# strongbeamsprout/gloria-nlp-project

Measured on AMD Instinct MI355X. Metric: image-text pairs/sec (whole node), imagenome_pretrain bs=256, higher is better.
Workload: dtype bf16

## Files before the change

### gloria-nlp-project_amd/csrc/glr_attn.hip

```cpp
#include "glr_attn_common.h"

namespace {

__global__ void __launch_bounds__(AT_NT) k_attn_fwd(AttnParams p) {
  extern __shared__ __attribute__((aligned(16))) unsigned char smem[];
  const int tid = threadIdx.x, lane = tid & 63, wave = tid >> 6, l31 = lane & 31, h = lane >> 5;
  const int bh = blockIdx.x, b = bh / p.nh, hd = bh % p.nh;
  int L; size_t row_base;
  attn_rows(p, b, row_base, L);
  const int tp = p.tp, lk = (L + 15) & ~15, kt = lk >> 4, nkb = (L + 31) >> 5;
  unsigned char* Qs = smem;
  unsigned char* Ks = Qs + 128 * AT_RP;
  unsigned char* Vt = Ks + 128 * AT_RP;
  unsigned char* Ps = smem;
  float* kb = reinterpret_cast<float*>(Vt + 64 * tp);
  const size_t base = row_base * p.ld + (size_t)hd * 64;
  {
    uint4 rq[4], rk[4], rv[4];
    tile_load(p.q + base, p.ld, L, rq, tid);
    tile_load(p.k + base, p.ld, L, rk, tid);
    tile_load(p.v + base, p.ld, L, rv, tid);
    tile_store_rows(rq, Qs, tid);
    tile_store_rows(rk, Ks, tid);
    tile_store_transposed(rv, lk, Vt, tp, tid);
  }
  if (tid < 128) kb[tid] = (tid < L && (p.key_mask == nullptr || p.key_mask[(size_t)b * L + tid] != 0)) ? 0.f : -INFINITY;
  __syncthreads();
  const int row0 = 32 * wave;
  f32x16 acc[4];
#pragma unroll
  for (int j = 0; j < 4; ++j) zero16(acc[j]);
  if (row0 < L) gemm_rows64(acc, Qs, row0, Ks, nkb, l31, h);
  __syncthreads();
  if (row0 >= L) return;
  float kbv[4];
#pragma unroll
  for (int j = 0; j < 4; ++j) kbv[j] = kb[32 * j + l31];
  const bool drop = p.p_drop > 0.f;
  const unsigned thr16 = drop ? (unsigned)(p.p_drop * 65536.f + 0.5f) : 0u;
  const float inv_keep = drop ? 1.f / (1.f - p.p_drop) : 1.f;
  const float sl = p.scale * AT_LOG2E;
  unsigned char* slab = Ps + wave * 32 * AT_SP;
  unsigned mw0 = 0u, mw1 = 0u;
  unsigned hk0, hk1;
  hash_key(p, hk0, hk1);
#pragma unroll
  for (int q = 0; q < 16; ++q) {
    const int r = acc_row(q, h);
    float v[4], m = -INFINITY;
#pragma unroll
    for (int j = 0; j < 4; ++j) { v[j] = __builtin_fmaf(acc[j][q], sl, kbv[j]); m = fmaxf(m, v[j]); }
    m = half_max(m);
    const float ms = m == -INFINITY ? 0.f : m;
    float e[4], s = 0.f;
#pragma unroll
    for (int j = 0; j < 4; ++j) { e[j] = __builtin_amdgcn_exp2f(v[j] - ms); s += e[j]; }
    s = half_sum(s);
    const float inv = s > 0.f ? 1.f / s : 0.f;
    if (l31 == 0) p.lse[(size_t)bh * 128 + row0 + r] = (ms + __builtin_amdgcn_logf(fmaxf(s, 1e-37f))) * (1.f / AT_LOG2E);
    unsigned r01 = 0u, r23 = 0u;
    if (drop) {
      const unsigned ctr = (((unsigned)bh * 128u + (unsigned)(row0 + r)) * 32u + (unsigned)l31) * 2u;
      r01 = hash32(ctr, hk0, hk1);
      r23 = hash32(ctr + 1u, hk0, hk1);
    }
    const unsigned r16[4] = {r01 & 0xffffu, r01 >> 16, r23 & 0xffffu, r23 >> 16};
#pragma unroll
    for (int j = 0; j < 4; ++j) {
      const bool keepb = !drop || r16[j] >= thr16;
      if (drop) {
        const unsigned long long word = __ballot(keepb);
        if (lane == q * 4 + j) { mw0 = (unsigned)word; mw1 = (unsigned)(word >> 32); }
      }
      const float pd = keepb ? e[j] * inv * inv_keep : 0.f;
      *reinterpret_cast<unsigned short*>(slab + r * AT_SP + (32 * j + l31) * 2) = f2bf(pd);
    }
  }
  if (drop) {
    const int q = lane >> 2, j = lane & 3;
    const int r0 = row0 + acc_row(q, 0);
    p.keep[((size_t)bh * 128 + r0) * 4 + j] = mw0;
    p.keep[((size_t)bh * 128 + r0 + 4) * 4 + j] = mw1;
  }
  f32x16 out[2];
  zero16(out[0]); zero16(out[1]);
  gemm_tokens(out, slab, Vt, tp, kt, l31, h);
  store_rows(out, slab, tp, p.o + row_base * p.ld_o + (size_t)hd * 64, p.ld_o, row0, L, lane, l31, h);
}

__global__ void __launch_bounds__(AT_NT, 2) k_attn_bwd_q(AttnParams p) {
  extern __shared__ __attribute__((aligned(16))) unsigned char smem[];
  const int tid = threadIdx.x, lane = tid & 63, wave = tid >> 6, l31 = lane & 31, h = lane >> 5;
  const int bh = blockIdx.x, b = bh / p.nh, hd = bh % p.nh;
  int L; size_t row_base;
  attn_rows(p, b, row_base, L);
  const int tp = p.tp, lk = (L + 15) & ~15, kt = lk >> 4, nkb = (L + 31) >> 5;
  unsigned char* Ks = smem;
  unsigned char* Vs = Ks + 128 * AT_RP;
  unsigned char* Kt = Vs + 128 * AT_RP;
  unsigned char* Ps = smem;
  float* kb = reinterpret_cast<float*>(Kt + 64 * tp);
  float* lse = kb + 128;
  float* delta = lse + 128;
  unsigned* keep = reinterpret_cast<unsigned*>(delta + 128);
  const size_t base = row_base * p.ld + (size_t)hd * 64, base_o = row_base * p.ld_o + (size_t)hd * 64;
  const bool drop = p.p_drop > 0.f;
  const int row0 = 32 * wave;
  const bool active = row0 < L;
  bf16x8 fq[4], fg[4];
  {
    uint4 rk[4], rv[4];
    bf16x8 fo[4];
    tile_load(p.k + base, p.ld, L, rk, tid);
    tile_load(p.v + base, p.ld, L, rv, tid);
    frag_rows_load(p.q + base, p.ld, row0 + l31, L, h, fq);
    frag_rows_load(p.d_o + base_o, p.ld_o, row0 + l31, L, h, fg);
    frag_rows_load(p.o + base_o, p.ld_o, row0 + l31, L, h, fo);
    if (tid < 128) {
      kb[tid] = (tid < L && (p.key_mask == nullptr || p.key_mask[(size_t)b * L + tid] != 0)) ? 0.f : -INFINITY;
      lse[tid] = tid < L ? p.lse[(size_t)bh * 128 + tid] * AT_LOG2E : 0.f;
    }
    for (int i = tid; i < 512; i += AT_NT) keep[i] = (drop && (i >> 2) < L) ? p.keep[(size_t)bh * 512 + i] : 0xffffffffu;
    tile_store_rows(rk, Ks, tid);
    tile_store_rows(rv, Vs, tid);
    tile_store_transposed(rk, lk, Kt, tp, tid);
    float d = 0.f;
#pragma unroll
    for (int ks = 0; ks < 4; ++ks) d += dot8(__builtin_bit_cast(uint4, fg[ks]), __builtin_bit_cast(uint4, fo[ks]));
    d += __shfl_xor(d, 32, 64);
    if (h == 0) delta[row0 + l31] = d;
  }
  __syncthreads();
  f32x16 acc[4], acc2[4], out[2];
#pragma unroll
  for (int j = 0; j < 4; ++j) { zero16(acc[j]); zero16(acc2[j]); }
  if (active) {
    gemm_frag64(acc, fq, Ks, nkb, l31, h);
    gemm_frag64(acc2, fg, Vs, nkb, l31, h);
  }
  __syncthreads();
  if (!active) return;
  const float inv_keep = drop ? 1.f / (1.f - p.p_drop) : 1.f;
  const float sl = p.scale * AT_LOG2E;
  unsigned char* slab = Ps + wave * 32 * AT_SP;
  {
    float kbv[4];
#pragma unroll
    for (int j = 0; j < 4; ++j) kbv[j] = kb[32 * j + l31];
#pragma unroll
    for (int q = 0; q < 16; ++q) {
      const int r = acc_row(q, h);
      const float lr = lse[row0 + r], dl = delta[row0 + r];
      const uint4 kw = *reinterpret_cast<const uint4*>(keep + (row0 + r) * 4);
      const unsigned kwj[4] = {kw.x, kw.y, kw.z, kw.w};
#pragma unroll
      for (int j = 0; j < 4; ++j) {
        const float pr = __builtin_amdgcn_exp2f(__builtin_fmaf(acc[j][q], sl, kbv[j]) - lr);
        const float dp = ((kwj[j] >> l31) & 1u) ? acc2[j][q] * inv_keep : 0.f;
        *reinterpret_cast<unsigned short*>(slab + r * AT_SP + (32 * j + l31) * 2) = f2bf(pr * (dp - dl) * p.scale);
      }
    }
  }
  zero16(out[0]); zero16(out[1]);
  gemm_tokens(out, slab, Kt, tp, kt, l31, h);
  store_rows(out, slab, tp, p.dq + base, p.ld, row0, L, lane, l31, h);
}

__global__ void __launch_bounds__(AT_NT, 2) k_attn_bwd_kv(AttnParams p) {
  extern __shared__ __attribute__((aligned(16))) unsigned char smem[];
  const int tid = threadIdx.x, lane = tid & 63, wave = tid >> 6, l31 = lane & 31, h = lane >> 5;
  const int bh = blockIdx.x, b = bh / p.nh, hd = bh % p.nh;
  int L; size_t row_base;
  attn_rows(p, b, row_base, L);
  const int tp = p.tp, lk = (L + 15) & ~15, kt = lk >> 4, nkb = (L + 31) >> 5;
  unsigned char* Qs = smem;
  unsigned char* Gs = Qs + 128 * AT_RP;
  unsigned char* Qt = Gs + 128 * AT_RP;
  unsigned char* Gt = Qt + 64 * tp;
  unsigned char* Ps = smem;
  float* kb = reinterpret_cast<float*>(Gt + 64 * tp);
  float* lse = kb + 128;
  float* delta = lse + 128;
  unsigned* keep = reinterpret_cast<unsigned*>(delta + 256);
  const size_t base = row_base * p.ld + (size_t)hd * 64, base_o = row_base * p.ld_o + (size_t)hd * 64;
  const bool drop = p.p_drop > 0.f;
  const int row0 = 32 * wave;
  const bool active = row0 < L;
  bf16x8 fk[4], fv[4];
  {
    uint4 rq[4], rg[4], ro[4];
    tile_load(p.q + base, p.ld, L, rq, tid);
    tile_load(p.d_o + base_o, p.ld_o, L, rg, tid);
    tile_load(p.o + base_o, p.ld_o, L, ro, tid);
    frag_rows_load(p.k + base, p.ld, row0 + l31, L, h, fk);
    frag_rows_load(p.v + base, p.ld, row0 + l31, L, h, fv);
    if (tid < 128) {
      kb[tid] = (tid < L && (p.key_mask == nullptr || p.key_mask[(size_t)b * L + tid] != 0)) ? 0.f : -INFINITY;
      lse[tid] = tid < L ? p.lse[(size_t)bh * 128 + tid] * AT_LOG2E : 0.f;
    }
    for (int i = tid; i < 512; i += AT_NT) keep[i] = (drop && (i >> 2) < L) ? p.keep[(size_t)bh * 512 + i] : 0xffffffffu;
    tile_store_rows(rq, Qs, tid);
    tile_store_rows(rg, Gs, tid);
    tile_store_transposed(rq, lk, Qt, tp, tid);
    tile_store_transposed(rg, lk, Gt, tp, tid);
    delta[tid] = (dot8(rg[0], ro[0]) + dot8(rg[1], ro[1])) + (dot8(rg[2], ro[2]) + dot8(rg[3], ro[3]));
  }
  __syncthreads();
  f32x16 acc[4], acc2[4], out[2];
#pragma unroll
  for (int j = 0; j < 4; ++j) { zero16(acc[j]); zero16(acc2[j]); }
  float lq[4], dq_[4], kbk16[16];
  unsigned kwq[4];
  if (active) {
    gemm_frag64(acc, fk, Qs, nkb, l31, h);
    gemm_frag64(acc2, fv, Gs, nkb, l31, h);
  }
#pragma unroll
  for (int j = 0; j < 4; ++j) {
    lq[j] = lse[32 * j + l31];
    dq_[j] = delta[32 * j + l31] + delta[128 + 32 * j + l31];
    kwq[j] = keep[(32 * j + l31) * 4 + wave];
  }
#pragma unroll
  for (int q = 0; q < 16; ++q) kbk16[q] = kb[row0 + acc_row(q, h)];
  __syncthreads();
  if (!active) return;
  const float inv_keep = drop ? 1.f / (1.f - p.p_drop) : 1.f;
  const float sl = p.scale * AT_LOG2E;
  unsigned char* slab = Ps + wave * 32 * AT_SP;
#pragma unroll
  for (int q = 0; q < 16; ++q) {
    const int r = acc_row(q, h);
#pragma unroll
    for (int j = 0; j < 4; ++j) {
      const float pr = __builtin_amdgcn_exp2f(__builtin_fmaf(acc[j][q], sl, kbk16[q]) - lq[j]);
      const bool keepb = (kwq[j] >> r) & 1u;
      *reinterpret_cast<unsigned short*>(slab + r * AT_SP + (32 * j + l31) * 2) = f2bf(keepb ? pr * inv_keep : 0.f);
      const float dp = keepb ? acc2[j][q] * inv_keep : 0.f;
      acc2[j][q] = pr * (dp - dq_[j]) * p.scale;
    }
  }
  zero16(out[0]); zero16(out[1]);
  gemm_tokens(out, slab, Gt, tp, kt, l31, h);
  {
    f32x16 dvv[2] = {out[0], out[1]};
#pragma unroll
    for (int q = 0; q < 16; ++q) {
      const int r = acc_row(q, h);
#pragma unroll
      for (int j = 0; j < 4; ++j) *reinterpret_cast<unsigned short*>(slab + r * AT_SP + (32 * j + l31) * 2) = f2bf(acc2[j][q]);
    }
    zero16(out[0]); zero16(out[1]);
    gemm_tokens(out, slab, Qt, tp, kt, l31, h);
    store_rows(out, slab, tp, p.dk + base, p.ld, row0, L, lane, l31, h);
    store_rows(dvv, slab, tp, p.dv + base, p.ld, row0, L, lane, l31, h);
  }
}

size_t attn_lds_fwd(int L) { return (size_t)2 * 128 * AT_RP + (size_t)64 * attn_tp(L) + 512; }
size_t attn_lds_bwd_q(int L) { return (size_t)2 * 128 * AT_RP + (size_t)64 * attn_tp(L) + 3 * 512 + 2048; }
size_t attn_lds_bwd_kv(int L) { return (size_t)2 * 128 * AT_RP + (size_t)2 * 64 * attn_tp(L) + 4 * 512 + 2048; }
size_t attn_lds_bwd(int L) { return attn_lds_bwd_kv(L) > attn_lds_bwd_q(L) ? attn_lds_bwd_kv(L) : attn_lds_bwd_q(L); }

}

extern "C" int glr_attn_max_tokens(int backward) {
  for (int L = 128; L > 0; L -= 16)
    if ((backward ? attn_lds_bwd(L) : attn_lds_fwd(L)) <= 160 * 1024) return L;
  return 0;
}

static int attn_launch_fwd(const AttnParams& p, void* stream) {
  const int lds = (int)attn_lds_fwd(p.L);
  static GlrLdsAttr lds_fwd;
  if (glr_ensure_lds(lds_fwd, (const void*)k_attn_fwd, lds) != GLR_OK) return GLR_ELAUNCH;
  hipLaunchKernelGGL(k_attn_fwd, dim3(p.B * p.nh), dim3(AT_NT), lds, (hipStream_t)stream, p);
  GLR_CHECK_LAUNCH();
  return GLR_OK;
}
static int attn_launch_bwd(const AttnParams& p, void* stream) {
  const int lds_q = (int)attn_lds_bwd_q(p.L), lds_kv = (int)attn_lds_bwd_kv(p.L);
  static GlrLdsAttr lds_bq, lds_bkv;
  if (glr_ensure_lds(lds_bq, (const void*)k_attn_bwd_q, lds_q) != GLR_OK) return GLR_ELAUNCH;
  if (glr_ensure_lds(lds_bkv, (const void*)k_attn_bwd_kv, lds_kv) != GLR_OK) return GLR_ELAUNCH;
  hipLaunchKernelGGL(k_attn_bwd_q, dim3(p.B * p.nh), dim3(AT_NT), lds_q, (hipStream_t)stream, p);
  GLR_CHECK_LAUNCH();
  hipLaunchKernelGGL(k_attn_bwd_kv, dim3(p.B * p.nh), dim3(AT_NT), lds_kv, (hipStream_t)stream, p);
  GLR_CHECK_LAUNCH();
  return GLR_OK;
}
static int attn_rows_longest(const int32_t* rs, int B, int max_n) {
  int longest = 0;
  for (int b = 0; b < B; ++b) {
    const long long n = (long long)rs[b + 1] - rs[b];
    if (rs[b] < 0 || n < 1 || n > max_n) return 0;
    if ((int)n > longest) longest = (int)n;
  }
  return longest;
}

extern "C" int glr_attn_fwd(const void* q, const void* k, const void* v, const uint8_t* key_mask, int B, int n_heads, int L, int ld,
                            int ld_o, float scale, float p_drop, unsigned long long seed, unsigned long long offset,
                            const unsigned long long* rng_cell, void* o, float* lse, uint32_t* keep, void* stream) {
  AttnParams p;
  const int rc = attn_fill(p, q, k, v, key_mask, B, n_heads, L, ld, ld_o, scale, p_drop, seed, offset, 128);
  if (rc != GLR_OK) return rc;
  if (!o || !lse || (p_drop > 0.f && !keep) || L > glr_attn_max_tokens(0)) return GLR_EINVAL;
  p.o = (unsigned short*)o; p.lse = lse; p.keep = keep; p.rng = rng_cell;
  return attn_launch_fwd(p, stream);
}

extern "C" int glr_attn_bwd(const void* q, const void* k, const void* v, const void* o, const void* d_o, const uint8_t* key_mask,
                            const float* lse, const uint32_t* keep, int B, int n_heads, int L, int ld, int ld_o, float scale, float p_drop,
                            void* dq, void* dk, void* dv, void* stream) {
  AttnParams p;
  const int rc = attn_fill(p, q, k, v, key_mask, B, n_heads, L, ld, ld_o, scale, p_drop, 0, 0, 128);
  if (rc != GLR_OK) return rc;
  if (!o || !d_o || !lse || !dq || !dk || !dv || (p_drop > 0.f && !keep) || L > glr_attn_max_tokens(1)) return GLR_EINVAL;
  p.o = (unsigned short*)const_cast<void*>(o); p.d_o = (const unsigned short*)d_o; p.lse = const_cast<float*>(lse);
  p.keep = const_cast<unsigned*>(keep); p.dq = (unsigned short*)dq; p.dk = (unsigned short*)dk; p.dv = (unsigned short*)dv;
  return attn_launch_bwd(p, stream);
}

extern "C" int glr_attn_rows_fwd(const void* q, const void* k, const void* v, const int32_t* row_start, const int32_t* row_start_host,
                                 int B, int n_heads, int ld, int ld_o, float scale, float p_drop, unsigned long long seed,
                                 unsigned long long offset, const unsigned long long* rng_cell, void* o, float* lse, uint32_t* keep,
                                 void* stream) {
  if (!row_start || !row_start_host || B <= 0) return GLR_EINVAL;
  const int longest = attn_rows_longest(row_start_host, B, glr_attn_max_tokens(0));
  if (longest == 0) return GLR_EINVAL;
  AttnParams p;
  const int rc = attn_fill(p, q, k, v, nullptr, B, n_heads, longest, ld, ld_o, scale, p_drop, seed, offset, 128);
  if (rc != GLR_OK) return rc;
  if (!o || !lse || (p_drop > 0.f && !keep)) return GLR_EINVAL;
  p.o = (unsigned short*)o; p.lse = lse; p.keep = keep; p.rng = rng_cell; p.row_start = row_start;
  return attn_launch_fwd(p, stream);
}

extern "C" int glr_attn_rows_bwd(const void* q, const void* k, const void* v, const void* o, const void* d_o, const int32_t* row_start,
                                 const int32_t* row_start_host, const float* lse, const uint32_t* keep, int B, int n_heads, int ld,
                                 int ld_o, float scale, float p_drop, void* dq, void* dk, void* dv, void* stream) {
  if (!row_start || !row_start_host || B <= 0) return GLR_EINVAL;
  const int longest = attn_rows_longest(row_start_host, B, glr_attn_max_tokens(1));
  if (longest == 0) return GLR_EINVAL;
  AttnParams p;
  const int rc = attn_fill(p, q, k, v, nullptr, B, n_heads, longest, ld, ld_o, scale, p_drop, 0, 0, 128);
  if (rc != GLR_OK) return rc;
  if (!o || !d_o || !lse || !dq || !dk || !dv || (p_drop > 0.f && !keep)) return GLR_EINVAL;
  p.o = (unsigned short*)const_cast<void*>(o); p.d_o = (const unsigned short*)d_o; p.lse = const_cast<float*>(lse);
  p.keep = const_cast<unsigned*>(keep); p.dq = (unsigned short*)dq; p.dk = (unsigned short*)dk; p.dv = (unsigned short*)dv;
  p.row_start = row_start;
  return attn_launch_bwd(p, stream);
}
```

### gloria-nlp-project_amd/csrc/glr_attn_common.h

```cpp
#pragma once
#include "glr_common.h"

namespace {

constexpr int AT_NT = 256;
constexpr int AT_RP = 144;
constexpr int AT_SP = 272;
constexpr float AT_LOG2E = 1.4426950408889634f;

struct AttnParams {
  const unsigned short* q; const unsigned short* k; const unsigned short* v;
  const unsigned char* key_mask;
  int B, nh, L, ld, ld_o;
  float scale, p_drop;
  unsigned seed_lo, seed_hi, off_lo, off_hi;
  const unsigned long long* rng;
  unsigned short* o;
  float* lse;
  unsigned* keep;
  const unsigned short* d_o;
  unsigned short* dq; unsigned short* dk; unsigned short* dv;
  int tp;
  const int* row_start;
};
// ... 40 lines not shown
  for (int q = 0; q < 16; ++q) a[q] = 0.f;
}
__device__ __forceinline__ int acc_row(int q, int h) { return (q & 3) + 8 * (q >> 2) + 4 * h; }

__device__ __forceinline__ void tile_load(const unsigned short* g, int ld, int L, uint4 (&r)[4], int tid) {
#pragma unroll
  for (int t = 0; t < 4; ++t) {
    const int i = tid + AT_NT * t, row = i & 127, pc = i >> 7;
    r[t] = make_uint4(0u, 0u, 0u, 0u);
    if (row < L) r[t] = *reinterpret_cast<const uint4*>(g + (size_t)row * ld + pc * 8);
  }
}
__device__ __forceinline__ void tile_store_rows(const uint4 (&r)[4], unsigned char* dst, int tid) {
#pragma unroll
  for (int t = 0; t < 4; ++t) {
    const int i = tid + AT_NT * t, row = i & 127, pc = i >> 7;
    *reinterpret_cast<uint4*>(dst + row * AT_RP + pc * 16) = r[t];
  }
}
__device__ __forceinline__ void tile_store_transposed(const uint4 (&r)[4], int lk, unsigned char* dst, int tp, int tid) {
#pragma unroll
  for (int t = 0; t < 4; ++t) {
    const int i = tid + AT_NT * t, row = i & 127, pc = i >> 7;
    if (row < lk) {
      const unsigned w[4] = {r[t].x, r[t].y, r[t].z, r[t].w};
#pragma unroll
      for (int e = 0; e < 4; ++e) {
        *reinterpret_cast<unsigned short*>(dst + (pc * 8 + 2 * e) * tp + row * 2) = (unsigned short)(w[e] & 0xffffu);
        *reinterpret_cast<unsigned short*>(dst + (pc * 8 + 2 * e + 1) * tp + row * 2) = (unsigned short)(w[e] >> 16);
      }
    }
  }
}
__device__ __forceinline__ float dot8(const uint4 a, const uint4 c) {
  const unsigned aw[4] = {a.x, a.y, a.z, a.w}, cw[4] = {c.x, c.y, c.z, c.w};
  float d = 0.f;
#pragma unroll
  for (int e = 0; e < 4; ++e) {
    d = __builtin_fmaf(__uint_as_float(aw[e] << 16), __uint_as_float(cw[e] << 16), d);
    d = __builtin_fmaf(__uint_as_float(aw[e] & 0xffff0000u), __uint_as_float(cw[e] & 0xffff0000u), d);
  }
  return d;
}
__device__ __forceinline__ void gemm_rows64(f32x16 (&acc)[4], const unsigned char* A, int arow0, const unsigned char* Bm, int nblk,
                                            int l31, int h) {
#pragma unroll
  for (int ks = 0; ks < 4; ++ks) {
    const bf16x8 fa = ldf(A + (arow0 + l31) * AT_RP + ks * 32 + h * 16);
#pragma unroll
    for (int j = 0; j < 4; ++j)
      if (j < nblk) mma(fa, ldf(Bm + (32 * j + l31) * AT_RP + ks * 32 + h * 16), acc[j]);
  }
}
__device__ __forceinline__ void gemm_tokens(f32x16 (&out)[2], const unsigned char* slab, const unsigned char* Bt, int tp, int kt,
                                            int l31, int h) {
  for (int ks = 0; ks < kt; ++ks) {
    const bf16x8 fa = ldf(slab + l31 * AT_SP + ks * 32 + h * 16);
#pragma unroll
    for (int c = 0; c < 2; ++c) mma(fa, ldf(Bt + (32 * c + l31) * tp + ks * 32 + h * 16), out[c]);
  }
}
__device__ __forceinline__ void store_rows(const f32x16 (&out)[2], unsigned char* slab, int tp, unsigned short* g, int ld, int row0, int L,
                                           int lane, int l31, int h) {
#pragma unroll
  for (int c = 0; c < 2; ++c)
#pragma unroll
// ... 53 lines not shown
```

### gloria-nlp-project_amd/csrc/glr_lnorm.hip

```cpp
#include "glr_common.h"

namespace {

constexpr int LN_NT = 256;

struct U4 { unsigned x, y, z, w; };
__device__ __forceinline__ U4 philox4x32(unsigned c0, unsigned c1, unsigned c2, unsigned c3, unsigned k0, unsigned k1) {
#pragma unroll
  for (int r = 0; r < 10; ++r) {
    const unsigned hi0 = __umulhi(0xD2511F53u, c0), lo0 = 0xD2511F53u * c0;
    const unsigned hi1 = __umulhi(0xCD9E8D57u, c2), lo1 = 0xCD9E8D57u * c2;
    c0 = hi1 ^ c1 ^ k0; c1 = lo1; c2 = hi0 ^ c3 ^ k1; c3 = lo0;
    k0 += 0x9E3779B9u; k1 += 0xBB67AE85u;
  }
  return {c0, c1, c2, c3};
}
__device__ __forceinline__ float wave_sum_f(float v) {
#pragma unroll
  for (int m = 32; m >= 1; m >>= 1) v += __shfl_xor(v, m, 64);
  return v;
}
__device__ __forceinline__ void unpack4(const uint2 u, float (&f)[4]) {
  f[0] = __uint_as_float(u.x << 16); f[1] = __uint_as_float(u.x & 0xffff0000u);
  f[2] = __uint_as_float(u.y << 16); f[3] = __uint_as_float(u.y & 0xffff0000u);
// ... 135 lines not shown
        dg[i][c] = __builtin_fmaf(dv[c], x, dg[i][c]);
        db[i][c] += dv[c];
      }
    }
    const float m1 = wave_sum_f(s1) * (1.f / H), m2 = wave_sum_f(s2) * (1.f / H);
#pragma unroll
    for (int i = 0; i < NQ; ++i) {
      const int quad = lane + 64 * i;
      float dz[4], dh[4];
#pragma unroll
      for (int c = 0; c < 4; ++c) {
        dz[c] = rstd * (gd[i][c] - m1 - xh[i][c] * m2);
        dh[c] = ((keepbits[i] >> c) & 1u) ? dz[c] * inv_keep : 0.f;
        dhs[i][c] += dh[c];
      }
      *reinterpret_cast<float4*>(d_inp + row * H + 4 * quad) = make_float4(dz[0], dz[1], dz[2], dz[3]);
      *reinterpret_cast<uint2*>(d_h + row * H + 4 * quad) = pack4(dh);
    }
  }
  __shared__ float red[3][LN_NT / 64][H];
#pragma unroll
  for (int i = 0; i < NQ; ++i)
#pragma unroll
    for (int c = 0; c < 4; ++c) {
      red[0][wv][4 * (lane + 64 * i) + c] = dg[i][c];
      red[1][wv][4 * (lane + 64 * i) + c] = db[i][c];
      red[2][wv][4 * (lane + 64 * i) + c] = dhs[i][c];
    }
  __syncthreads();
  for (int col = threadIdx.x; col < H; col += LN_NT) {
    float a = 0.f, b = 0.f, e = 0.f;
#pragma unroll
    for (int k = 0; k < LN_NT / 64; ++k) { a += red[0][k][col]; b += red[1][k][col]; e += red[2][k][col]; }
    part[(size_t)col * gridDim.x + blockIdx.x] = a;
    part[((size_t)H + col) * gridDim.x + blockIdx.x] = b;
    part[((size_t)2 * H + col) * gridDim.x + blockIdx.x] = e;
  }
}

__global__ void __launch_bounds__(LN_NT) k_ln_finish(const float* __restrict__ part, int n_part, int H, float* __restrict__ dgamma,
                                                     float* __restrict__ dbeta, void* __restrict__ dhsum, int dhsum_bf16) {
  const int lane = threadIdx.x & 63;
  const int col = blockIdx.x * (LN_NT / 64) + (threadIdx.x >> 6);
  if (col >= H) return;
  float a = 0.f, b = 0.f, e = 0.f;
  for (int k = lane; k < n_part; k += 64) {
    a += part[(size_t)col * n_part + k];
    b += part[((size_t)H + col) * n_part + k];
    if (dhsum) e += part[((size_t)2 * H + col) * n_part + k];
  }
  a = wave_sum_f(a);
  b = wave_sum_f(b);
  e = wave_sum_f(e);
  if (lane == 0) {
    dgamma[col] = a;
    dbeta[col] = b;
    if (dhsum) {
      if (dhsum_bf16) reinterpret_cast<unsigned short*>(dhsum)[col] = f2bf(e);
      else reinterpret_cast<float*>(dhsum)[col] = e;
    }
  }
}

constexpr int CS_COLS = 256;
__global__ void __launch_bounds__(LN_NT) k_colsum(const unsigned short* __restrict__ x, long long R, int C, long long rows_per,
                                                   float* __restrict__ part) {
  const int ct = threadIdx.x & 31, rl = threadIdx.x >> 5;
  const int col0 = blockIdx.x * CS_COLS + ct * 8;
  const long long r0 = (long long)blockIdx.y * rows_per;
  const long long r1 = r0 + rows_per < R ? r0 + rows_per : R;
  float acc[8] = {0.f, 0.f, 0.f, 0.f, 0.f, 0.f, 0.f, 0.f};
  const unsigned short* px = x + col0;
  long long r = r0 + rl;
  for (; r + 24 < r1; r += 32) {
    uint4 v[4];
#pragma unroll
    for (int u = 0; u < 4; ++u) v[u] = *reinterpret_cast<const uint4*>(px + (r + 8 * u) * C);
#pragma unroll
    for (int u = 0; u < 4; ++u) {
      acc[0] += __uint_as_float(v[u].x << 16); acc[1] += __uint_as_float(v[u].x & 0xffff0000u);
      acc[2] += __uint_as_float(v[u].y << 16); acc[3] += __uint_as_float(v[u].y & 0xffff0000u);
      acc[4] += __uint_as_float(v[u].z << 16); acc[5] += __uint_as_float(v[u].z & 0xffff0000u);
      acc[6] += __uint_as_float(v[u].w << 16); acc[7] += __uint_as_float(v[u].w & 0xffff0000u);
    }
  }
  for (; r < r1; r += 8) {
    const uint4 v = *reinterpret_cast<const uint4*>(px + r * C);
    acc[0] += __uint_as_float(v.x << 16); acc[1] += __uint_as_float(v.x & 0xffff0000u);
    acc[2] += __uint_as_float(v.y << 16); acc[3] += __uint_as_float(v.y & 0xffff0000u);
    acc[4] += __uint_as_float(v.z << 16); acc[5] += __uint_as_float(v.z & 0xffff0000u);
    acc[6] += __uint_as_float(v.w << 16); acc[7] += __uint_as_float(v.w & 0xffff0000u);
  }
  __shared__ float red[8][CS_COLS + 8];
#pragma unroll
// ... 79 lines not shown
                                   unsigned long long* mask, void* stream) {
  return drop_add_ln_fwd(h16, inp32, gamma, beta, R, H, eps, p_drop, seed, offset, rng_cell, out32, out16, stats, mask, nullptr, stream);
}

extern "C" int glr_drop_add_ln_rows_fwd(const void* h16, const float* inp32, const float* gamma, const float* beta,
                                        const int32_t* row_ids, long long R, int H, float eps, float p_drop, unsigned long long seed,
                                        unsigned long long offset, const unsigned long long* rng_cell, float* out32, void* out16,
                                        float* stats, unsigned long long* mask, void* stream) {
  if (!row_ids) return GLR_EINVAL;
  return drop_add_ln_fwd(h16, inp32, gamma, beta, R, H, eps, p_drop, seed, offset, rng_cell, out32, out16, stats, mask, row_ids, stream);
}

extern "C" int glr_drop_add_ln_bwd(const float* dy32, const void* dy16, const void* h16, const float* inp32, const float* gamma,
                                   const float* stats, const unsigned long long* mask, long long R, int H, float p_drop,
                                   float* d_inp32, void* d_h16, float* workspace, float* dgamma, float* dbeta, void* dhsum,
                                   int dhsum_bf16, void* stream) {
  if ((!dy32 && !dy16) || !h16 || !inp32 || !gamma || !stats || !d_inp32 || !d_h16 || !workspace || !dgamma || !dbeta ||
      !ln_shape_ok(R, H))
    return GLR_EINVAL;
  if (p_drop < 0.f || p_drop >= 1.f || (p_drop > 0.f && !mask)) return GLR_EINVAL;
  hipStream_t st = (hipStream_t)stream;
  const int np = ln_parts(R);
#define GLR_LN_BWD(NQ)                                                                                                      \
  hipLaunchKernelGGL((k_drop_add_ln_bwd<NQ>), dim3(np), dim3(LN_NT), 0, st, dy32, (const unsigned short*)dy16,               \
                     (const unsigned short*)h16, inp32, gamma, stats, mask, R, p_drop, d_inp32, (unsigned short*)d_h16, workspace)
  switch (H / 256) {
    case 1: GLR_LN_BWD(1); break;
    case 2: GLR_LN_BWD(2); break;
    case 3: GLR_LN_BWD(3); break;
    default: GLR_LN_BWD(4); break;
  }
#undef GLR_LN_BWD
  GLR_CHECK_LAUNCH();
  hipLaunchKernelGGL(k_ln_finish, dim3((H + LN_NT / 64 - 1) / (LN_NT / 64)), dim3(LN_NT), 0, st, workspace, np, H, dgamma, dbeta, dhsum,
                     dhsum_bf16);
  GLR_CHECK_LAUNCH();
  return GLR_OK;
}
```

Baseline: 4102.

## Pack multiple short-sequence heads per attention block and restructure LN finish reduction

Attention forward and backward kernels now pack several heads into one 128-row block when the sequence is short (<=32 or <=64 tokens), using templated bodies that skip unused key blocks. This cuts idle waves and shrinks the grid for short text sequences. Separately, the layernorm-backward partials are stored row-major per block, and the finish kernel is rewritten as a column-coalesced 1024-thread reduction. The head packing adds index arithmetic and shared-memory layout complexity.

Result: slower. 4039 (-1.5%).

```diff
diff --git a/gloria-nlp-project_amd/csrc/glr_attn.hip b/gloria-nlp-project_amd/csrc/glr_attn.hip
--- a/gloria-nlp-project_amd/csrc/glr_attn.hip
+++ b/gloria-nlp-project_amd/csrc/glr_attn.hip
@@ -2,40 +2,66 @@
 
 namespace {
 
-__global__ void __launch_bounds__(AT_NT) k_attn_fwd(AttnParams p) {
-  extern __shared__ __attribute__((aligned(16))) unsigned char smem[];
+struct AttnUnit {
+  int hd, bh, hl, R0, row0, L, lk, kt, nkb, tp;
+  bool active;
+};
+__device__ __forceinline__ AttnUnit attn_unit(const AttnParams& p, int b, int hd0, int nhg, int sh, int L, int tp, int wave) {
+  AttnUnit u;
+  u.L = L; u.tp = tp;
+  u.R0 = 32 * wave; u.hl = u.R0 >> sh; u.row0 = u.R0 & ((1 << sh) - 1);
+  u.hd = hd0 + u.hl; u.bh = b * p.nh + u.hd;
+  u.lk = (L + 15) & ~15; u.kt = u.lk >> 4; u.nkb = (L + 31) >> 5;
+  u.active = u.hl < nhg && u.row0 < L;
+  return u;
+}
+__device__ __forceinline__ bool attn_group(const AttnParams& p, int G, int& b, int& hd0, int& nhg, int& sh, int& L, size_t& row_base, int& tp) {
+  b = blockIdx.x / G;
+  attn_rows(p, b, row_base, L);
+  sh = L <= 32 ? 5 : (L <= 64 ? 6 : 7);
+  const int hpw = 128 >> sh;
+  hd0 = (blockIdx.x % G) * hpw;
+  nhg = p.nh - hd0 < hpw ? p.nh - hd0 : hpw;
+  tp = (2 << sh) + 16;
+  return hd0 < p.nh;
+}
+
+template <int SH>
+__device__ __forceinline__ void attn_fwd_body(const AttnParams& p, unsigned char* smem, int b, int hd0, int nhg, int L_,
+                                              size_t row_base, int tp_) {
   const int tid = threadIdx.x, lane = tid & 63, wave = tid >> 6, l31 = lane & 31, h = lane >> 5;
-  const int bh = blockIdx.x, b = bh / p.nh, hd = bh % p.nh;
-  int L; size_t row_base;
-  attn_rows(p, b, row_base, L);
-  const int tp = p.tp, lk = (L + 15) & ~15, kt = lk >> 4, nkb = (L + 31) >> 5;
+  const AttnUnit u = attn_unit(p, b, hd0, nhg, SH, L_, tp_, wave);
+  constexpr int NKB = SH == 5 ? 1 : (SH == 6 ? 2 : 4);
+  const int L = u.L, tp = u.tp, lk = u.lk, kt = u.kt, nkb = NKB < 4 ? NKB : u.nkb, sh = SH, bh = u.bh, hd = u.hd;
   unsigned char* Qs = smem;
   unsigned char* Ks = Qs + 128 * AT_RP;
   unsigned char* Vt = Ks + 128 * AT_RP;
   unsigned char* Ps = smem;
-  float* kb = reinterpret_cast<float*>(Vt + 64 * tp);
-  const size_t base = row_base * p.ld + (size_t)hd * 64;
+  float* kb = reinterpret_cast<float*>(Vt + (64 * tp << (7 - sh)));
+  const size_t base = row_base * p.ld + (size_t)hd0 * 64;
   {
     uint4 rq[4], rk[4], rv[4];
-    tile_load(p.q + base, p.ld, L, rq, tid);
-    tile_load(p.k + base, p.ld, L, rk, tid);
-    tile_load(p.v + base, p.ld, L, rv, tid);
+    tile_load_group(p.q + base, p.ld, L, sh, nhg, rq, tid);
+    tile_load_group(p.k + base, p.ld, L, sh, nhg, rk, tid);
+    tile_load_group(p.v + base, p.ld, L, sh, nhg, rv, tid);
     tile_store_rows(rq, Qs, tid);
     tile_store_rows(rk, Ks, tid);
-    tile_store_transposed(rv, lk, Vt, tp, tid);
+    tile_store_transposed_group(rv, lk, Vt, tp, sh, tid);
   }
   if (tid < 128) kb[tid] = (tid < L && (p.key_mask == nullptr || p.key_mask[(size_t)b * L + tid] != 0)) ? 0.f : -INFINITY;
   __syncthreads();
-  const int row0 = 32 * wave;
+  Ks += (u.hl << sh) * AT_RP;
+  Vt += (size_t)u.hl * 64 * tp;
+  const int row0 = u.row0;
   f32x16 acc[4];
 #pragma unroll
   for (int j = 0; j < 4; ++j) zero16(acc[j]);
-  if (row0 < L) gemm_rows64(acc, Qs, row0, Ks, nkb, l31, h);
-  __syncthreads();
-  if (row0 >= L) return;
+  if (u.active) gemm_rows64(acc, Qs, u.R0, Ks, nkb, l31, h);
+  __syncthreads();
+  if (!u.active) return;
   float kbv[4];
 #pragma unroll
-  for (int j = 0; j < 4; ++j) kbv[j] = kb[32 * j + l31];
+  for (int j = 0; j < 4; ++j) kbv[j] = j < NKB ? kb[32 * j + l31] : -INFINITY;
   const bool drop = p.p_drop > 0.f;
   const unsigned thr16 = drop ? (unsigned)(p.p_drop * 65536.f + 0.5f) : 0u;
   const float inv_keep = drop ? 1.f / (1.f - p.p_drop) : 1.f;
@@ -49,12 +75,14 @@
     const int r = acc_row(q, h);
     float v[4], m = -INFINITY;
 #pragma unroll
-    for (int j = 0; j < 4; ++j) { v[j] = __builtin_fmaf(acc[j][q], sl, kbv[j]); m = fmaxf(m, v[j]); }
+    for (int j = 0; j < 4; ++j)
+      if (j < NKB) { v[j] = __builtin_fmaf(acc[j][q], sl, kbv[j]); m = fmaxf(m, v[j]); }
     m = half_max(m);
     const float ms = m == -INFINITY ? 0.f : m;
     float e[4], s = 0.f;
 #pragma unroll
-    for (int j = 0; j < 4; ++j) { e[j] = __builtin_amdgcn_exp2f(v[j] - ms); s += e[j]; }
+    for (int j = 0; j < 4; ++j)
+      if (j < NKB) { e[j] = __builtin_amdgcn_exp2f(v[j] - ms); s += e[j]; }
     s = half_sum(s);
     const float inv = s > 0.f ? 1.f / s : 0.f;
     if (l31 == 0) p.lse[(size_t)bh * 128 + row0 + r] = (ms + __builtin_amdgcn_logf(fmaxf(s, 1e-37f))) * (1.f / AT_LOG2E);
@@ -72,8 +100,10 @@
         const unsigned long long word = __ballot(keepb);
         if (lane == q * 4 + j) { mw0 = (unsigned)word; mw1 = (unsigned)(word >> 32); }
       }
-      const float pd = keepb ? e[j] * inv * inv_keep : 0.f;
-      *reinterpret_cast<unsigned short*>(slab + r * AT_SP + (32 * j + l31) * 2) = f2bf(pd);
+      if (j < NKB) {
+        const float pd = keepb ? e[j] * inv * inv_keep : 0.f;
+        *reinterpret_cast<unsigned short*>(slab + r * AT_SP + (32 * j + l31) * 2) = f2bf(pd);
+      }
     }
   }
   if (drop) {
@@ -88,49 +118,74 @@
   store_rows(out, slab, tp, p.o + row_base * p.ld_o + (size_t)hd * 64, p.ld_o, row0, L, lane, l31, h);
 }
 
-__global__ void __launch_bounds__(AT_NT, 2) k_attn_bwd_q(AttnParams p) {
-  extern __shared__ __attribute__((aligned(16))) unsigned char smem[];
-  const int tid = threadIdx.x, lane = tid & 63, wave = tid >> 6, l31 = lane & 31, h = lane >> 5;
-  const int bh = blockIdx.x, b = bh / p.nh, hd = bh % p.nh;
+__global__ void __launch_bounds__(AT_NT) k_attn_fwd(AttnParams p) {
+  extern __shared__ __attribute__((aligned(16))) unsigned char smem[];
+  const int b = blockIdx.x / p.nh, hd = blockIdx.x % p.nh;
   int L; size_t row_base;
   attn_rows(p, b, row_base, L);
-  const int tp = p.tp, lk = (L + 15) & ~15, kt = lk >> 4, nkb = (L + 31) >> 5;
+  attn_fwd_body<7>(p, smem, b, hd, 1, L, row_base, p.tp);
+}
+__global__ void __launch_bounds__(AT_NT) k_attn_units_fwd(AttnParams p, int G) {
+  extern __shared__ __attribute__((aligned(16))) unsigned char smem[];
+  int b, hd0, nhg, sh, L, tp; size_t row_base;
+  if (!attn_group(p, G, b, hd0, nhg, sh, L, row_base, tp)) return;
+  if (sh == 5) attn_fwd_body<5>(p, smem, b, hd0, nhg, L, row_base, tp);
+  else if (sh == 6) attn_fwd_body<6>(p, smem, b, hd0, nhg, L, row_base, tp);
+  else attn_fwd_body<7>(p, smem, b, hd0, nhg, L, row_base, tp);
+}
+
+template <int SH>
+__device__ __forceinline__ void attn_bwd_q_body(const AttnParams& p, unsigned char* smem, int b, int hd0, int nhg, int L_,
+                                                size_t row_base, int tp_) {
+  const int tid = threadIdx.x, lane = tid & 63, wave = tid >> 6, l31 = lane & 31, h = lane >> 5;
+  const AttnUnit u = attn_unit(p, b, hd0, nhg, SH, L_, tp_, wave);
+  constexpr int NKB = SH == 5 ? 1 : (SH == 6 ? 2 : 4);
+  const int L = u.L, tp = u.tp, lk = u.lk, kt = u.kt, nkb = NKB < 4 ? NKB : u.nkb, sh = SH;
   unsigned char* Ks = smem;
   unsigned char* Vs = Ks + 128 * AT_RP;
   unsigned char* Kt = Vs + 128 * AT_RP;
   unsigned char* Ps = smem;
-  float* kb = reinterpret_cast<float*>(Kt + 64 * tp);
+  float* kb = reinterpret_cast<float*>(Kt + (64 * tp << (7 - sh)));
   float* lse = kb + 128;
   float* delta = lse + 128;
   unsigned* keep = reinterpret_cast<unsigned*>(delta + 128);
-  const size_t base = row_base * p.ld + (size_t)hd * 64, base_o = row_base * p.ld_o + (size_t)hd * 64;
+  const size_t base0 = row_base * p.ld + (size_t)hd0 * 64;
+  const size_t base = row_base * p.ld + (size_t)u.hd * 64, base_o = row_base * p.ld_o + (size_t)u.hd * 64;
   const bool drop = p.p_drop > 0.f;
-  const int row0 = 32 * wave;
-  const bool active = row0 < L;
+  const int row0 = u.row0, R0 = u.R0;
+  const int Lw = u.hl < nhg ? L : 0;
+  const bool active = u.active;
   bf16x8 fq[4], fg[4];
   {
     uint4 rk[4], rv[4];
     bf16x8 fo[4];
-    tile_load(p.k + base, p.ld, L, rk, tid);
-    tile_load(p.v + base, p.ld, L, rv, tid);
-    frag_rows_load(p.q + base, p.ld, row0 + l31, L, h, fq);
-    frag_rows_load(p.d_o + base_o, p.ld_o, row0 + l31, L, h, fg);
-    frag_rows_load(p.o + base_o, p.ld_o, row0 + l31, L, h, fo);
+    tile_load_group(p.k + base0, p.ld, L, sh, nhg, rk, tid);
+    tile_load_group(p.v + base0, p.ld, L, sh, nhg, rv, tid);
+    frag_rows_load(p.q + base, p.ld, row0 + l31, Lw, h, fq);
+    frag_rows_load(p.d_o + base_o, p.ld_o, row0 + l31, Lw, h, fg);
+    frag_rows_load(p.o + base_o, p.ld_o, row0 + l31, Lw, h, fo);
     if (tid < 128) {
+      const int hl = tid >> sh, tok = tid & ((1 << sh) - 1);
       kb[tid] = (tid < L && (p.key_mask == nullptr || p.key_mask[(size_t)b * L + tid] != 0)) ? 0.f : -INFINITY;
-      lse[tid] = tid < L ? p.lse[(size_t)bh * 128 + tid] * AT_LOG2E : 0.f;
-    }
-    for (int i = tid; i < 512; i += AT_NT) keep[i] = (drop && (i >> 2) < L) ? p.keep[(size_t)bh * 512 + i] : 0xffffffffu;
+      lse[tid] = (tok < L && hl < nhg) ? p.lse[(size_t)(b * p.nh + hd0 + hl) * 128 + tok] * AT_LOG2E : 0.f;
+    }
+    for (int i = tid; i < 512; i += AT_NT) {
+      const int hl = (i >> 2) >> sh, tok = (i >> 2) & ((1 << sh) - 1);
+      keep[i] = (drop && tok < L && hl < nhg) ? p.keep[(size_t)(b * p.nh + hd0 + hl) * 512 + tok * 4 + (i & 3)] : 0xffffffffu;
+    }
     tile_store_rows(rk, Ks, tid);
     tile_store_rows(rv, Vs, tid);
-    tile_store_transposed(rk, lk, Kt, tp, tid);
+    tile_store_transposed_group(rk, lk, Kt, tp, sh, tid);
     float d = 0.f;
 #pragma unroll
     for (int ks = 0; ks < 4; ++ks) d += dot8(__builtin_bit_cast(uint4, fg[ks]), __builtin_bit_cast(uint4, fo[ks]));
     d += __shfl_xor(d, 32, 64);
-    if (h == 0) delta[row0 + l31] = d;
-  }
-  __syncthreads();
+    if (h == 0) delta[R0 + l31] = d;
+  }
+  __syncthreads();
+  Ks += (u.hl << sh) * AT_RP;
+  Vs += (u.hl << sh) * AT_RP;
+  Kt += (size_t)u.hl * 64 * tp;
   f32x16 acc[4], acc2[4], out[2];
 #pragma unroll
   for (int j = 0; j < 4; ++j) { zero16(acc[j]); zero16(acc2[j]); }
@@ -146,66 +201,92 @@
   {
     float kbv[4];
 #pragma unroll
-    for (int j = 0; j < 4; ++j) kbv[j] = kb[32 * j + l31];
+    for (int j = 0; j < 4; ++j) kbv[j] = j < NKB ? kb[32 * j + l31] : -INFINITY;
 #pragma unroll
     for (int q = 0; q < 16; ++q) {
       const int r = acc_row(q, h);
-      const float lr = lse[row0 + r], dl = delta[row0 + r];
-      const uint4 kw = *reinterpret_cast<const uint4*>(keep + (row0 + r) * 4);
+      const float lr = lse[R0 + r], dl = delta[R0 + r];
+      const uint4 kw = *reinterpret_cast<const uint4*>(keep + (R0 + r) * 4);
       const unsigned kwj[4] = {kw.x, kw.y, kw.z, kw.w};
 #pragma unroll
-      for (int j = 0; j < 4; ++j) {
-        const float pr = __builtin_amdgcn_exp2f(__builtin_fmaf(acc[j][q], sl, kbv[j]) - lr);
-        const float dp = ((kwj[j] >> l31) & 1u) ? acc2[j][q] * inv_keep : 0.f;
-        *reinterpret_cast<unsigned short*>(slab + r * AT_SP + (32 * j + l31) * 2) = f2bf(pr * (dp - dl) * p.scale);
-      }
+      for (int j = 0; j < 4; ++j)
+        if (j < NKB) {
+          const float pr = __builtin_amdgcn_exp2f(__builtin_fmaf(acc[j][q], sl, kbv[j]) - lr);
+          const float dp = ((kwj[j] >> l31) & 1u) ? acc2[j][q] * inv_keep : 0.f;
+          *reinterpret_cast<unsigned short*>(slab + r * AT_SP + (32 * j + l31) * 2) = f2bf(pr * (dp - dl) * p.scale);
+        }
     }
   }
   zero16(out[0]); zero16(out[1]);
   gemm_tokens(out, slab, Kt, tp, kt, l31, h);
   store_rows(out, slab, tp, p.dq + base, p.ld, row0, L, lane, l31, h);
 }
-
-__global__ void __launch_bounds__(AT_NT, 2) k_attn_bwd_kv(AttnParams p) {
-  extern __shared__ __attribute__((aligned(16))) unsigned char smem[];
-  const int tid = threadIdx.x, lane = tid & 63, wave = tid >> 6, l31 = lane & 31, h = lane >> 5;
-  const int bh = blockIdx.x, b = bh / p.nh, hd = bh % p.nh;
+__global__ void __launch_bounds__(AT_NT, 2) k_attn_bwd_q(AttnParams p) {
+  extern __shared__ __attribute__((aligned(16))) unsigned char smem[];
+  const int b = blockIdx.x / p.nh, hd = blockIdx.x % p.nh;
   int L; size_t row_base;
   attn_rows(p, b, row_base, L);
-  const int tp = p.tp, lk = (L + 15) & ~15, kt = lk >> 4, nkb = (L + 31) >> 5;
+  attn_bwd_q_body<7>(p, smem, b, hd, 1, L, row_base, p.tp);
+}
+__global__ void __launch_bounds__(AT_NT, 2) k_attn_units_bwd_q(AttnParams p, int G) {
+  extern __shared__ __attribute__((aligned(16))) unsigned char smem[];
+  int b, hd0, nhg, sh, L, tp; size_t row_base;
+  if (!attn_group(p, G, b, hd0, nhg, sh, L, row_base, tp)) return;
+  if (sh == 5) attn_bwd_q_body<5>(p, smem, b, hd0, nhg, L, row_base, tp);
+  else if (sh == 6) attn_bwd_q_body<6>(p, smem, b, hd0, nhg, L, row_base, tp);
+  else attn_bwd_q_body<7>(p, smem, b, hd0, nhg, L, row_base, tp);
+}
+
+template <int SH>
+__device__ __forceinline__ void attn_bwd_kv_body(const AttnParams& p, unsigned char* smem, int b, int hd0, int nhg, int L_,
+                                                 size_t row_base, int tp_) {
+  const int tid = threadIdx.x, lane = tid & 63, wave = tid >> 6, l31 = lane & 31, h = lane >> 5;
+  const AttnUnit u = attn_unit(p, b, hd0, nhg, SH, L_, tp_, wave);
+  constexpr int NKB = SH == 5 ? 1 : (SH == 6 ? 2 : 4);
+  const int L = u.L, tp = u.tp, lk = u.lk, kt = u.kt, nkb = NKB < 4 ? NKB : u.nkb, sh = SH;
   unsigned char* Qs = smem;
   unsigned char* Gs = Qs + 128 * AT_RP;
   unsigned char* Qt = Gs + 128 * AT_RP;
-  unsigned char* Gt = Qt + 64 * tp;
+  unsigned char* Gt = Qt + (64 * tp << (7 - sh));
   unsigned char* Ps = smem;
-  float* kb = reinterpret_cast<float*>(Gt + 64 * tp);
+  float* kb = reinterpret_cast<float*>(Gt + (64 * tp << (7 - sh)));
   float* lse = kb + 128;
   float* delta = lse + 128;
   unsigned* keep = reinterpret_cast<unsigned*>(delta + 256);
-  const size_t base = row_base * p.ld + (size_t)hd * 64, base_o = row_base * p.ld_o + (size_t)hd * 64;
+  const size_t base0 = row_base * p.ld + (size_t)hd0 * 64, base0_o = row_base * p.ld_o + (size_t)hd0 * 64;
+  const size_t base = row_base * p.ld + (size_t)u.hd * 64;
   const bool drop = p.p_drop > 0.f;
-  const int row0 = 32 * wave;
-  const bool active = row0 < L;
+  const int row0 = u.row0, Rh = u.hl << sh;
+  const int Lw = u.hl < nhg ? L : 0;
+  const bool active = u.active;
   bf16x8 fk[4], fv[4];
   {
     uint4 rq[4], rg[4], ro[4];
-    tile_load(p.q + base, p.ld, L, rq, tid);
-    tile_load(p.d_o + base_o, p.ld_o, L, rg, tid);
-    tile_load(p.o + base_o, p.ld_o, L, ro, tid);
-    frag_rows_load(p.k + base, p.ld, row0 + l31, L, h, fk);
-    frag_rows_load(p.v + base, p.ld, row0 + l31, L, h, fv);
+    tile_load_group(p.q + base0, p.ld, L, sh, nhg, rq, tid);
+    tile_load_group(p.d_o + base0_o, p.ld_o, L, sh, nhg, rg, tid);
+    tile_load_group(p.o + base0_o, p.ld_o, L, sh, nhg, ro, tid);
+    frag_rows_load(p.k + base, p.ld, row0 + l31, Lw, h, fk);
+    frag_rows_load(p.v + base, p.ld, row0 + l31, Lw, h, fv);
     if (tid < 128) {
+      const int hl = tid >> sh, tok = tid & ((1 << sh) - 1);
       kb[tid] = (tid < L && (p.key_mask == nullptr || p.key_mask[(size_t)b * L + tid] != 0)) ? 0.f : -INFINITY;
-      lse[tid] = tid < L ? p.lse[(size_t)bh * 128 + tid] * AT_LOG2E : 0.f;
-    }
-    for (int i = tid; i < 512; i += AT_NT) keep[i] = (drop && (i >> 2) < L) ? p.keep[(size_t)bh * 512 + i] : 0xffffffffu;
+      lse[tid] = (tok < L && hl < nhg) ? p.lse[(size_t)(b * p.nh + hd0 + hl) * 128 + tok] * AT_LOG2E : 0.f;
+    }
+    for (int i = tid; i < 512; i += AT_NT) {
+      const int hl = (i >> 2) >> sh, tok = (i >> 2) & ((1 << sh) - 1);
+      keep[i] = (drop && tok < L && hl < nhg) ? p.keep[(size_t)(b * p.nh + hd0 + hl) * 512 + tok * 4 + (i & 3)] : 0xffffffffu;
+    }
     tile_store_rows(rq, Qs, tid);
     tile_store_rows(rg, Gs, tid);
-    tile_store_transposed(rq, lk, Qt, tp, tid);
-    tile_store_transposed(rg, lk, Gt, tp, tid);
+    tile_store_transposed_group(rq, lk, Qt, tp, sh, tid);
+    tile_store_transposed_group(rg, lk, Gt, tp, sh, tid);
     delta[tid] = (dot8(rg[0], ro[0]) + dot8(rg[1], ro[1])) + (dot8(rg[2], ro[2]) + dot8(rg[3], ro[3]));
   }
   __syncthreads();
+  Qs += Rh * AT_RP;
+  Gs += Rh * AT_RP;
+  Qt += (size_t)u.hl * 64 * tp;
+  Gt += (size_t)u.hl * 64 * tp;
   f32x16 acc[4], acc2[4], out[2];
 #pragma unroll
   for (int j = 0; j < 4; ++j) { zero16(acc[j]); zero16(acc2[j]); }
@@ -217,9 +298,12 @@
   }
 #pragma unroll
   for (int j = 0; j < 4; ++j) {
-    lq[j] = lse[32 * j + l31];
-    dq_[j] = delta[32 * j + l31] + delta[128 + 32 * j + l31];
-    kwq[j] = keep[(32 * j + l31) * 4 + wave];
+    lq[j] = 0.f; dq_[j] = 0.f; kwq[j] = 0u;
+    if (j < NKB) {
+      lq[j] = lse[Rh + 32 * j + l31];
+      dq_[j] = delta[Rh + 32 * j + l31] + delta[128 + Rh + 32 * j + l31];
+      kwq[j] = keep[(Rh + 32 * j + l31) * 4 + (row0 >> 5)];
+    }
   }
 #pragma unroll
   for (int q = 0; q < 16; ++q) kbk16[q] = kb[row0 + acc_row(q, h)];
@@ -232,13 +316,14 @@
   for (int q = 0; q < 16; ++q) {
     const int r = acc_row(q, h);
 #pragma unroll
-    for (int j = 0; j < 4; ++j) {
-      const float pr = __builtin_amdgcn_exp2f(__builtin_fmaf(acc[j][q], sl, kbk16[q]) - lq[j]);
-      const bool keepb = (kwq[j] >> r) & 1u;
-      *reinterpret_cast<unsigned short*>(slab + r * AT_SP + (32 * j + l31) * 2) = f2bf(keepb ? pr * inv_keep : 0.f);
-      const float dp = keepb ? acc2[j][q] * inv_keep : 0.f;
-      acc2[j][q] = pr * (dp - dq_[j]) * p.scale;
-    }
+    for (int j = 0; j < 4; ++j)
+      if (j < NKB) {
+        const float pr = __builtin_amdgcn_exp2f(__builtin_fmaf(acc[j][q], sl, kbk16[q]) - lq[j]);
+        const bool keepb = (kwq[j] >> r) & 1u;
+        *reinterpret_cast<unsigned short*>(slab + r * AT_SP + (32 * j + l31) * 2) = f2bf(keepb ? pr * inv_keep : 0.f);
+        const float dp = keepb ? acc2[j][q] * inv_keep : 0.f;
+        acc2[j][q] = pr * (dp - dq_[j]) * p.scale;
+      }
   }
   zero16(out[0]); zero16(out[1]);
   gemm_tokens(out, slab, Gt, tp, kt, l31, h);
@@ -248,7 +333,8 @@
     for (int q = 0; q < 16; ++q) {
       const int r = acc_row(q, h);
 #pragma unroll
-      for (int j = 0; j < 4; ++j) *reinterpret_cast<unsigned short*>(slab + r * AT_SP + (32 * j + l31) * 2) = f2bf(acc2[j][q]);
+      for (int j = 0; j < 4; ++j)
+        if (j < NKB) *reinterpret_cast<unsigned short*>(slab + r * AT_SP + (32 * j + l31) * 2) = f2bf(acc2[j][q]);
     }
     zero16(out[0]); zero16(out[1]);
     gemm_tokens(out, slab, Qt, tp, kt, l31, h);
@@ -256,6 +342,26 @@
     store_rows(dvv, slab, tp, p.dv + base, p.ld, row0, L, lane, l31, h);
   }
 }
+__global__ void __launch_bounds__(AT_NT, 2) k_attn_bwd_kv(AttnParams p) {
+  extern __shared__ __attribute__((aligned(16))) unsigned char smem[];
+  const int b = blockIdx.x / p.nh, hd = blockIdx.x % p.nh;
+  int L; size_t row_base;
+  attn_rows(p, b, row_base, L);
+  attn_bwd_kv_body<7>(p, smem, b, hd, 1, L, row_base, p.tp);
+}
+__global__ void __launch_bounds__(AT_NT, 2) k_attn_units_bwd_kv(AttnParams p, int G) {
+  extern __shared__ __attribute__((aligned(16))) unsigned char smem[];
+  int b, hd0, nhg, sh, L, tp; size_t row_base;
+  if (!attn_group(p, G, b, hd0, nhg, sh, L, row_base, tp)) return;
+  if (sh == 5) attn_bwd_kv_body<5>(p, smem, b, hd0, nhg, L, row_base, tp);
+  else if (sh == 6) attn_bwd_kv_body<6>(p, smem, b, hd0, nhg, L, row_base, tp);
+  else attn_bwd_kv_body<7>(p, smem, b, hd0, nhg, L, row_base, tp);
+}
+
+constexpr size_t AT_UNITS_T = 4 * 64 * 80;
+size_t attn_lds_units_fwd() { return (size_t)2 * 128 * AT_RP + AT_UNITS_T + 512; }
+size_t attn_lds_units_bwd_q() { return (size_t)2 * 128 * AT_RP + AT_UNITS_T + 3 * 512 + 2048; }
+size_t attn_lds_units_bwd_kv() { return (size_t)2 * 128 * AT_RP + 2 * AT_UNITS_T + 4 * 512 + 2048; }
 
 size_t attn_lds_fwd(int L) { return (size_t)2 * 128 * AT_RP + (size_t)64 * attn_tp(L) + 512; }
 size_t attn_lds_bwd_q(int L) { return (size_t)2 * 128 * AT_RP + (size_t)64 * attn_tp(L) + 3 * 512 + 2048; }
@@ -286,6 +392,29 @@
   hipLaunchKernelGGL(k_attn_bwd_q, dim3(p.B * p.nh), dim3(AT_NT), lds_q, (hipStream_t)stream, p);
   GLR_CHECK_LAUNCH();
   hipLaunchKernelGGL(k_attn_bwd_kv, dim3(p.B * p.nh), dim3(AT_NT), lds_kv, (hipStream_t)stream, p);
+  GLR_CHECK_LAUNCH();
+  return GLR_OK;
+}
+static int attn_units_groups(int nh, int longest) {
+  const int hpw = longest <= 32 ? 4 : (longest <= 64 ? 2 : 1);
+  return (nh + hpw - 1) / hpw;
+}
+static int attn_launch_units_fwd(const AttnParams& p, void* stream) {
+  const int lds = (int)attn_lds_units_fwd(), G = attn_units_groups(p.nh, p.L);
+  static GlrLdsAttr lds_fwd;
+  if (glr_ensure_lds(lds_fwd, (const void*)k_attn_units_fwd, lds) != GLR_OK) return GLR_ELAUNCH;
+  hipLaunchKernelGGL(k_attn_units_fwd, dim3(p.B * G), dim3(AT_NT), lds, (hipStream_t)stream, p, G);
+  GLR_CHECK_LAUNCH();
+  return GLR_OK;
+}
+static int attn_launch_units_bwd(const AttnParams& p, void* stream) {
+  const int lds_q = (int)attn_lds_units_bwd_q(), lds_kv = (int)attn_lds_units_bwd_kv(), G = attn_units_groups(p.nh, p.L);
+  static GlrLdsAttr lds_bq, lds_bkv;
+  if (glr_ensure_lds(lds_bq, (const void*)k_attn_units_bwd_q, lds_q) != GLR_OK) return GLR_ELAUNCH;
+  if (glr_ensure_lds(lds_bkv, (const void*)k_attn_units_bwd_kv, lds_kv) != GLR_OK) return GLR_ELAUNCH;
+  hipLaunchKernelGGL(k_attn_units_bwd_q, dim3(p.B * G), dim3(AT_NT), lds_q, (hipStream_t)stream, p, G);
+  GLR_CHECK_LAUNCH();
+  hipLaunchKernelGGL(k_attn_units_bwd_kv, dim3(p.B * G), dim3(AT_NT), lds_kv, (hipStream_t)stream, p, G);
   GLR_CHECK_LAUNCH();
   return GLR_OK;
 }
@@ -334,7 +463,7 @@
   if (rc != GLR_OK) return rc;
   if (!o || !lse || (p_drop > 0.f && !keep)) return GLR_EINVAL;
   p.o = (unsigned short*)o; p.lse = lse; p.keep = keep; p.rng = rng_cell; p.row_start = row_start;
-  return attn_launch_fwd(p, stream);
+  return attn_launch_units_fwd(p, stream);
 }
 
 extern "C" int glr_attn_rows_bwd(const void* q, const void* k, const void* v, const void* o, const void* d_o, const int32_t* row_start,
@@ -350,5 +479,5 @@
   p.o = (unsigned short*)const_cast<void*>(o); p.d_o = (const unsigned short*)d_o; p.lse = const_cast<float*>(lse);
   p.keep = const_cast<unsigned*>(keep); p.dq = (unsigned short*)dq; p.dk = (unsigned short*)dk; p.dv = (unsigned short*)dv;
   p.row_start = row_start;
-  return attn_launch_bwd(p, stream);
-}
+  return attn_launch_units_bwd(p, stream);
+}
diff --git a/gloria-nlp-project_amd/csrc/glr_attn_common.h b/gloria-nlp-project_amd/csrc/glr_attn_common.h
--- a/gloria-nlp-project_amd/csrc/glr_attn_common.h
+++ b/gloria-nlp-project_amd/csrc/glr_attn_common.h
@@ -96,6 +96,29 @@
     }
   }
 }
+__device__ __forceinline__ void tile_load_group(const unsigned short* g, int ld, int L, int sh, int nhg, uint4 (&r)[4], int tid) {
+#pragma unroll
+  for (int t = 0; t < 4; ++t) {
+    const int i = tid + AT_NT * t, R = i & 127, pc = i >> 7, hl = R >> sh, tok = R & ((1 << sh) - 1);
+    r[t] = make_uint4(0u, 0u, 0u, 0u);
+    if (tok < L && hl < nhg) r[t] = *reinterpret_cast<const uint4*>(g + (size_t)tok * ld + hl * 64 + pc * 8);
+  }
+}
+__device__ __forceinline__ void tile_store_transposed_group(const uint4 (&r)[4], int lk, unsigned char* dst, int tp, int sh, int tid) {
+#pragma unroll
+  for (int t = 0; t < 4; ++t) {
+    const int i = tid + AT_NT * t, R = i & 127, pc = i >> 7, hl = R >> sh, tok = R & ((1 << sh) - 1);
+    if (tok < lk) {
+      unsigned char* d = dst + (size_t)hl * 64 * tp;
+      const unsigned w[4] = {r[t].x, r[t].y, r[t].z, r[t].w};
+#pragma unroll
+      for (int e = 0; e < 4; ++e) {
+        *reinterpret_cast<unsigned short*>(d + (pc * 8 + 2 * e) * tp + tok * 2) = (unsigned short)(w[e] & 0xffffu);
+        *reinterpret_cast<unsigned short*>(d + (pc * 8 + 2 * e + 1) * tp + tok * 2) = (unsigned short)(w[e] >> 16);
+      }
+    }
+  }
+}
 __device__ __forceinline__ float dot8(const uint4 a, const uint4 c) {
   const unsigned aw[4] = {a.x, a.y, a.z, a.w}, cw[4] = {c.x, c.y, c.z, c.w};
   float d = 0.f;
diff --git a/gloria-nlp-project_amd/csrc/glr_lnorm.hip b/gloria-nlp-project_amd/csrc/glr_lnorm.hip
--- a/gloria-nlp-project_amd/csrc/glr_lnorm.hip
+++ b/gloria-nlp-project_amd/csrc/glr_lnorm.hip
@@ -191,34 +191,56 @@
     float a = 0.f, b = 0.f, e = 0.f;
 #pragma unroll
     for (int k = 0; k < LN_NT / 64; ++k) { a += red[0][k][col]; b += red[1][k][col]; e += red[2][k][col]; }
-    part[(size_t)col * gridDim.x + blockIdx.x] = a;
-    part[((size_t)H + col) * gridDim.x + blockIdx.x] = b;
-    part[((size_t)2 * H + col) * gridDim.x + blockIdx.x] = e;
-  }
-}
-
-__global__ void __launch_bounds__(LN_NT) k_ln_finish(const float* __restrict__ part, int n_part, int H, float* __restrict__ dgamma,
+    float* mine = part + (size_t)blockIdx.x * (3 * H);
+    mine[col] = a;
+    mine[H + col] = b;
+    mine[2 * H + col] = e;
+  }
+}
+
+constexpr int LF_NT = 1024, LF_COLS = 32, LF_LANES = 64 / (LF_NT / LF_COLS);
+__global__ void __launch_bounds__(LF_NT) k_ln_finish(const float* __restrict__ part, int n_part, int H, float* __restrict__ dgamma,
                                                      float* __restrict__ dbeta, void* __restrict__ dhsum, int dhsum_bf16) {
-  const int lane = threadIdx.x & 63;
-  const int col = blockIdx.x * (LN_NT / 64) + (threadIdx.x >> 6);
-  if (col >= H) return;
-  float a = 0.f, b = 0.f, e = 0.f;
-  for (int k = lane; k < n_part; k += 64) {
-    a += part[(size_t)col * n_part + k];
-    b += part[((size_t)H + col) * n_part + k];
-    if (dhsum) e += part[((size_t)2 * H + col) * n_part + k];
-  }
-  a = wave_sum_f(a);
-  b = wave_sum_f(b);
-  e = wave_sum_f(e);
-  if (lane == 0) {
-    dgamma[col] = a;
-    dbeta[col] = b;
-    if (dhsum) {
-      if (dhsum_bf16) reinterpret_cast<unsigned short*>(dhsum)[col] = f2bf(e);
-      else reinterpret_cast<float*>(dhsum)[col] = e;
-    }
-  }
+  const int c = threadIdx.x % LF_COLS, g = threadIdx.x / LF_COLS;
+  const int col3 = blockIdx.x * LF_COLS + c;
+  const int which = (blockIdx.x * LF_COLS) / H, col = col3 - which * H;
+  if (which == 2 && !dhsum) return;
+  float acc[LF_LANES];
+#pragma unroll
+  for (int i = 0; i < LF_LANES; ++i) acc[i] = 0.f;
+  const float* src = part + col3;
+  for (int k0 = 0; k0 < n_part; k0 += 256) {
+    float v[4][LF_LANES];
+#pragma unroll
+    for (int u = 0; u < 4; ++u)
+#pragma unroll
+      for (int i = 0; i < LF_LANES; ++i) {
+        const int k = k0 + 64 * u + LF_LANES * g + i;
+        v[u][i] = k < n_part ? src[(size_t)k * (3 * H)] : 0.f;
+      }
+#pragma unroll
+    for (int u = 0; u < 4; ++u)
+#pragma unroll
+      for (int i = 0; i < LF_LANES; ++i)
+        if (k0 + 64 * u + LF_LANES * g + i < n_part) acc[i] += v[u][i];
+  }
+  __shared__ float red[64][LF_COLS];
+#pragma unroll
+  for (int i = 0; i < LF_LANES; ++i) red[LF_LANES * g + i][c] = acc[i];
+  __syncthreads();
+  if (g != 0) return;
+  float v[32];
+#pragma unroll
+  for (int l = 0; l < 32; ++l) v[l] = red[l][c] + red[l + 32][c];
+#pragma unroll
+  for (int m = 16; m >= 1; m >>= 1)
+#pragma unroll
+    for (int l = 0; l < m; ++l) v[l] = v[l] + v[l + m];
+  const float a = v[0];
+  if (which == 0) dgamma[col] = a;
+  else if (which == 1) dbeta[col] = a;
+  else if (dhsum_bf16) reinterpret_cast<unsigned short*>(dhsum)[col] = f2bf(a);
+  else reinterpret_cast<float*>(dhsum)[col] = a;
 }
 
 constexpr int CS_COLS = 256;
@@ -364,8 +386,7 @@
   }
 #undef GLR_LN_BWD
   GLR_CHECK_LAUNCH();
-  hipLaunchKernelGGL(k_ln_finish, dim3((H + LN_NT / 64 - 1) / (LN_NT / 64)), dim3(LN_NT), 0, st, workspace, np, H, dgamma, dbeta, dhsum,
-                     dhsum_bf16);
+  hipLaunchKernelGGL(k_ln_finish, dim3(3 * H / LF_COLS), dim3(LF_NT), 0, st, workspace, np, H, dgamma, dbeta, dhsum, dhsum_bf16);
   GLR_CHECK_LAUNCH();
   return GLR_OK;
 }
```
